# GStreamer/gst-plugins-rs

Measured on AMD Instinct MI355X. Metric: 4K RGBA frames/sec through hsvfilter+colorlut at 1 GPU; % HBM roofline, higher is better.
Workload: dtype u8

## Files before the change

gst-plugins-rs_amd/csrc/colorlut_kernels.hip:

```cpp
#include "internal.hpp"
#include "hsv_device.hpp"
#include "exact_math.hpp"

#include <cmath>
#include <cstring>
#include <map>
#include <memory>
#include <mutex>
#include <vector>

namespace mi355 {

struct LutK {
  float scale[3];
  float offset[3];
  int size;
};


__device__ __forceinline__ uint32_t floor_idx(float x, uint32_t max_idx) {
  const float f = floorf(x);
  uint32_t i = (f > 0.0f) ? ((f >= 4294967040.0f) ? 0xffffffffu : (uint32_t)f) : 0u;
  return i < max_idx ? i : max_idx;
}
// ... 825 lines not shown
  __shared__ uint32_t s_strip[4][512];
  s_spread[threadIdx.x] = spread3(threadIdx.x);
  __syncthreads();
  auto index = [&](uint32_t p) -> uint32_t { return s_spread[p & 0xffu] | (s_spread[(p >> 8) & 0xffu] << 1) | (s_spread[(p >> 16) & 0xffu] << 2); };
  const unsigned wave = threadIdx.x >> 6, lane = threadIdx.x & 63;
  uint32_t *x = s_strip[wave];
  const unsigned frame = blockIdx.x / tiles_per_frame, t = blockIdx.x - frame * tiles_per_frame;
  const u32x4_t *s4 = (const u32x4_t *)srcs.p[frame];
  u32x4_t *d4 = (u32x4_t *)dsts.p[frame];
  auto wave_sync = [] {
    __builtin_amdgcn_fence(__ATOMIC_ACQ_REL, "wavefront");
    __builtin_amdgcn_wave_barrier();
  };
  constexpr unsigned RPL = 64 / TW4;
  const unsigned sub = lane / TW4, g = lane % TW4;
  const unsigned tx = t % n_cols, ty = t / n_cols;
  const unsigned col = tx * TW4 + g;
  const unsigned r0 = ty * (8 * RPL) + wave * (2 * RPL) + sub, r1 = r0 + RPL;
  const bool ok0 = col < w4 && r0 < rows, ok1 = col < w4 && r1 < rows;
  const size_t i0 = (size_t)r0 * w4 + col, i1 = (size_t)r1 * w4 + col;
  u32x4_t p = {0, 0, 0, 0}, q = {0, 0, 0, 0};
  if (ok0) p = __builtin_nontemporal_load(s4 + i0);
  if (ok1) q = __builtin_nontemporal_load(s4 + i1);
  *(u32x4_t *)(x + lane * 4) = p;
  *(u32x4_t *)(x + 256 + lane * 4) = q;
  wave_sync();
  uint32_t px[8], o[8];
#pragma unroll
  for (int j = 0; j < 8; j++) px[j] = x[j * 64 + lane];
#pragma unroll
  for (int j = 0; j < 8; j++) o[j] = table[index(px[j])];
#pragma unroll
  for (int j = 0; j < 8; j++) x[j * 64 + lane] = (o[j] & 0x00ffffffu) | (px[j] & 0xff000000u);
  wave_sync();
  const u32x4_t r0v = *(u32x4_t *)(x + lane * 4), r1v = *(u32x4_t *)(x + 256 + lane * 4);
  if (ok0) __builtin_nontemporal_store(r0v, d4 + i0);
  if (ok1) __builtin_nontemporal_store(r1v, d4 + i1);
}

void shared_table_release(mi355_ctx *ctx, std::shared_ptr<void> *ref);
void lut_release(mi355_ctx *ctx) {
  for (int i = 0; i < 2; i++) {
    shared_table_release(ctx, &ctx->lut.table_ref[i]);
    if (ctx->lut.pick[i].ev0) (void)hipEventDestroy(ctx->lut.pick[i].ev0);
    if (ctx->lut.pick[i].ev1) (void)hipEventDestroy(ctx->lut.pick[i].ev1);
  }
// ... 713 lines not shown
  MultiFramePtrs s{}, d{};
  for (int f = 0; f < n_frames; f++) {
    if (!srcs[f] || !dsts[f] || (uintptr_t)srcs[f] % 16 != 0 || (uintptr_t)dsts[f] % 16 != 0) return MI355_ERR_UNSUPPORTED;
    s.p[f] = srcs[f];
    d.p[f] = dsts[f];
  }
  const unsigned w4 = (unsigned)width / 4;
  if (from_hbm && ctx->lut_variant == 0 && window_multi_applicable(ctx, w4, (size_t)height, n_frames)) {
    ctx->lut.last_kernel = "colorlut_window_kernel";
    return launch_window_table_multi(ctx, stream, table, srcs, dsts, n_frames, w4, (size_t)height);
  }
  ctx->lut.last_kernel = "colorlut_table_tiled_multi_kernel";
  const unsigned pad64 = (w4 + 63) / 64 * 64 - w4, pad32 = (w4 + 31) / 32 * 32 - w4;
  const unsigned tw4 = pad64 <= pad32 ? 64 : 32;
  const unsigned n_cols = (w4 + tw4 - 1) / tw4, rpb = 8 * (64 / tw4);
  const size_t tiles_per_frame = (size_t)n_cols * (((size_t)height + rpb - 1) / rpb);
  const size_t grid = tiles_per_frame * (size_t)n_frames;
  if (grid >= (1u << 31)) return MI355_ERR_UNSUPPORTED;
  if (tw4 == 64) hipLaunchKernelGGL((colorlut_table_tiled_multi_kernel<64>), dim3((unsigned)grid), dim3(256), 0, stream, s, d, w4, (unsigned)height, n_cols, (unsigned)tiles_per_frame, table);
  else hipLaunchKernelGGL((colorlut_table_tiled_multi_kernel<32>), dim3((unsigned)grid), dim3(256), 0, stream, s, d, w4, (unsigned)height, n_cols, (unsigned)tiles_per_frame, table);
  return check_hip(ctx, hipGetLastError(), "colorlut multi-frame table kernel launch");
}

void hsv_table_release(mi355_ctx *ctx) {
  HsvTable &T = ctx->hsv_table;
  shared_table_release(ctx, &T.table_ref);
  if (T.pick.ev0) (void)hipEventDestroy(T.pick.ev0);
  if (T.pick.ev1) (void)hipEventDestroy(T.pick.ev1);
  T = HsvTable{};
}

static int hsv_table_ensure(mi355_ctx *ctx, const PixFmt &fmt, const mi355_hsv_settings &hs) {
  HsvTable &T = ctx->hsv_table;
  if (T.valid && T.bgr == fmt.bgr && same_hs(T.hs, hs)) return MI355_OK;
  T.valid = false;
  T.d_table = nullptr;
  std::string key("H");
  key.push_back((char)('0' + fmt.bgr));
  key.append((const char *)&hs, sizeof(hs));
  int rc = shared_table_acquire(ctx, key, &T.table_ref, &T.d_table, [&](uint32_t *tab) {
    hipLaunchKernelGGL(table_domain_kernel, dim3(kTableEntries / 256), dim3(256), 0, ctx->stream, tab, 1);
    return launch_hsvfilter_compute(ctx, (uint8_t *)tab, 1, 0, 4096, 4096, 4096 * 4, fmt, hs);
  });
  if (rc) { T.table_ref.reset(); T.d_table = nullptr; return rc; }
  T.valid = true;
  T.bgr = fmt.bgr;
// ... 67 lines not shown
```

gst-plugins-rs_amd/csrc/group.hip:

```cpp
#include "internal.hpp"

#include <chrono>
#include <condition_variable>
#include <algorithm>
#include <cstring>
#include <deque>
#include <mutex>
#include <unordered_map>
#include <vector>

using namespace mi355;

namespace {

struct Desc {
  mi355_ctx *ctx;
  uint8_t *src, *dst;
  int width, height, stride, format;
  mi355_hsv_settings hs;
  const uint32_t *table;
  std::shared_ptr<void> table_ref;
  bool batchable;
  bool fused;
  uint64_t ticket;
// ... 715 lines not shown
    for (Set &s : sets) {
      (void)hipEventDestroy(s.done);
      kind.blocks.give(&s.data.block);
    }
    sets.clear();
    for (Item &d : pending)
      if (d.ready) (void)hipEventDestroy(d.ready);
    pending.clear();
    kind.destroy();
  }
};

}

struct mi355_group : GroupCore {
  int max_batch = 8;
  hipStream_t stream = nullptr;
  std::vector<Desc> pending;
  std::deque<Batch> batches;
  std::unordered_map<uint64_t, uint64_t> where;
  std::unordered_map<uint64_t, int> failed;
  uint64_t next_seq = 1;
  uint64_t n_frames = 0, n_batched_launch_pairs = 0, n_single = 0;
  std::vector<std::shared_ptr<void>> dead_refs;
  SetQueue<CmpKind> cmp;
  SetQueue<CdKind> cd;
  SetQueue<HdKind> hd;
  SetQueue<YdKind> yd;
  SetQueue<HnKind> hn;
  SetQueue<HfKind> hf;
};

namespace {

struct Locked {
  std::vector<std::shared_ptr<void>> reap;
  mi355_group *g;
  std::unique_lock<std::mutex> lk;
  explicit Locked(mi355_group *g_) : g(g_), lk(g_->mu) {}
  ~Locked() {
    if (!lk.owns_lock()) lk.lock();
    reap.swap(g->dead_refs);
    lk.unlock();
  }
};

void retire_front(mi355_group *g) {
  Batch &b = g->batches.front();
  for (uint64_t t : b.tickets) g->where.erase(t);
  g->events.push_back(b.done);
  if (b.table_ref) g->dead_refs.push_back(std::move(b.table_ref));
  g->batches.pop_front();
}

void retire_done(mi355_group *g) {
  while (!g->batches.empty() && g->batches.front().waiters == 0) {
    if (hipEventQuery(g->batches.front().done) != hipSuccess) { (void)hipGetLastError(); break; }
    retire_front(g);
  }
}

bool same_class(const Desc &a, const Desc &b) {
  return a.batchable && b.batchable && a.fused == b.fused && a.width == b.width && a.height == b.height && a.stride == b.stride && a.format == b.format && a.table == b.table &&
         std::memcmp(&a.hs, &b.hs, sizeof(a.hs)) == 0 && a.ctx->force_generic == b.ctx->force_generic;
}

int flush_locked(mi355_group *g, uint64_t until = 0) {
  bool reached = false;
  while (!g->pending.empty() && !reached) {
    std::vector<Desc> take, keep;
    std::vector<mi355_ctx *> blocked;
    const Desc first = g->pending.front();
    for (const Desc &d : g->pending) {
      bool stream_blocked = false;
      for (mi355_ctx *c : blocked) stream_blocked |= c == d.ctx;
      const bool fits = take.empty() || (!stream_blocked && (int)take.size() < g->max_batch && same_class(first, d));
      if (fits) take.push_back(d);
      else keep.push_back(d);
      if (!stream_blocked) blocked.push_back(d.ctx);
    }
    g->pending.swap(keep);
    PixFmt fmt;
    (void)pixfmt_of(first.format, &fmt);
    hipEvent_t done = take_event(g);
    if (!done) return fail(g, MI355_ERR_HIP, "hipEventCreate");
    int rc = MI355_OK;
    if (first.batchable) {
      uint8_t *srcs[kMultiFrames], *dsts[kMultiFrames];
      for (size_t i = 0; i < take.size(); i++) {
        srcs[i] = take[i].src;
        dsts[i] = take[i].dst;
        if (take[i].ready && hipStreamWaitEvent(g->stream, take[i].ready, 0) != hipSuccess) rc = MI355_ERR_HIP;
      }
      if (!rc && !first.fused) rc = launch_hsvfilter_multi(first.ctx, g->stream, srcs, (int)take.size(), first.width, first.height, fmt, first.hs);
      if (!rc) rc = launch_colorlut_multi(first.ctx, g->stream, first.table, srcs, dsts, (int)take.size(), first.width, first.height, first.fused);
      if (!rc && hipEventRecord(done, g->stream) != hipSuccess) rc = MI355_ERR_HIP;
      g->n_batched_launch_pairs++;
    } else {
      const Desc &d = take[0];
      const size_t pitch = (size_t)d.stride * (size_t)d.height;
      if (!g->batches.empty() && hipStreamWaitEvent(d.ctx->stream, g->batches.back().done, 0) != hipSuccess) rc = MI355_ERR_HIP;
      if (!rc && d.fused) rc = launch_hsv_colorlut(d.ctx, d.src, pitch, d.stride, d.dst, pitch, d.stride, 1, d.width, d.height, d.hs);
      if (!rc && !d.fused) rc = launch_hsvfilter(d.ctx, d.src, 1, pitch, d.width, d.height, d.stride, fmt, d.hs);
      if (!rc && !d.fused) rc = launch_colorlut(d.ctx, d.src, pitch, d.stride, d.dst, pitch, d.stride, 1, d.width, d.height, d.format);
      if (!rc && hipEventRecord(done, d.ctx->stream) != hipSuccess) rc = MI355_ERR_HIP;
      if (!rc && hipStreamWaitEvent(g->stream, done, 0) != hipSuccess) rc = MI355_ERR_HIP;
      if (rc && rc != MI355_ERR_HIP) g->last_error = d.ctx->last_error;
      g->n_single++;
    }
    for (const Desc &d : take)
      if (d.ready) g->events.push_back(d.ready);
    if (rc) {
      (void)hipGetLastError();
      g->events.push_back(done);
      if (g->failed.size() > 65536) g->failed.clear();
      for (const Desc &d : take) g->failed[d.ticket] = rc;
      if (g->last_error.empty()) g->last_error = "group launch failed";
      return rc;
// ... 572 lines not shown
  }
  return mi355_group_flush(g);
}

int mi355_group_submit_round_fused(mi355_group *g, mi355_ctx *const *ctxs, int n_streams, uint8_t *const *d_src, uint8_t *const *d_dst, int width,
                                   int height, int stride, int format, const mi355_hsv_settings *settings) {
  if (!g || !ctxs || !d_src || !d_dst || n_streams < 0) return MI355_ERR_INVALID_ARG;
  for (int i = 0; i < n_streams; i++) {
    int rc = mi355_group_submit_fused(g, ctxs[i], d_src[i], d_dst[i], width, height, stride, format, settings, nullptr);
    if (rc) return rc;
  }
  return mi355_group_flush(g);
}

int mi355_group_stats(mi355_group *g, uint64_t stats[3]) {
  if (!g || !stats) return MI355_ERR_INVALID_ARG;
  std::lock_guard<std::mutex> lk(g->mu);
  stats[0] = g->n_frames;
  stats[1] = g->n_batched_launch_pairs;
  stats[2] = g->n_single;
  return MI355_OK;
}

}

namespace {
std::mutex g_pg_mu;
struct ProcessGroup { int device; mi355_group *g; int refs; };
std::vector<ProcessGroup> g_pg;
}

extern "C" {

mi355_group *mi355_group_shared(int device, int *status) {
  std::lock_guard<std::mutex> lk(g_pg_mu);
  for (ProcessGroup &p : g_pg)
    if (p.device == device) { p.refs++; if (status) *status = MI355_OK; return p.g; }
  mi355_group *g = mi355_group_create(device, 0, status);
  if (g) g_pg.push_back(ProcessGroup{device, g, 1});
  return g;
}

void mi355_group_release(mi355_group *g) {
  if (!g) return;
  bool last = false;
  {
// ... 13 lines not shown
```

gst-plugins-rs_amd/csrc/hsv_device.hpp:

```cpp
#pragma once
#include "internal.hpp"
#include "exact_math.hpp"

namespace mi355 {

struct HsvK {
  float hue_shift, sat_mul, sat_off, val_mul, val_off;
};


template <bool FAST>
__device__ __forceinline__ void hsv_from_rgb(float r8, float g8, float b8, float &hue, float &sat,
                                             float &val) {
  if constexpr (FAST) {
    const float r = div255_u8(r8), g = div255_u8(g8), b = div255_u8(b8);
    const float value = fmaxf(fmaxf(r, g), b);
    const float minv = fminf(fminf(r, g), b);
    const float chroma = value - minv;
    const bool is_r = (r == value);
    const bool is_g = (g == value);
    const float na = is_r ? g : (is_g ? b : r);
    const float nb = is_r ? b : (is_g ? r : g);
    const float add = is_r ? 0.0f : (is_g ? 2.0f : 4.0f);
    const float q = div_rcp_refine(na - nb, fmaxf(chroma, 1e-30f));
// ... 289 lines not shown
    r = (r >= 360.0f) ? r - 360.0f : r;
    return __builtin_copysignf(r, t);
  }
  return fmodf(t, 360.0f);
}
template <int RPOS, int GPOS, int BPOS, int NPOS>
__device__ __forceinline__ void hsvfilter_px2_generic(uint32_t &p0, uint32_t &p1, const HsvK &k, const HsvLds *lds) {
  f2 h2, sat, value;
  hsv_from_rgb_pair_fast<RPOS, GPOS, BPOS, 1>(p0, p1, h2, sat, value, lds);
  uint32_t *px[2] = {&p0, &p1};
#pragma unroll
  for (int j = 0; j < 2; j++) {
    float h = hsv_fmod360_any((j ? h2.y : h2.x) + k.hue_shift);
    if (h < 0.0f) h += 360.0f;
    const float s = fminf(fmaxf(k.sat_mul * (j ? sat.y : sat.x) + k.sat_off, 0.0f), 1.0f);
    const float v = fminf(fmaxf(k.val_mul * (j ? value.y : value.x) + k.val_off, 0.0f), 1.0f);
    uint32_t r, g, b;
    hsv_to_rgb_generic(h, s, v, r, g, b);
    const uint32_t keep = *px[j] & (0xffu << (8 * NPOS));
    *px[j] = keep | (r << (8 * RPOS)) | (g << (8 * GPOS)) | (b << (8 * BPOS));
  }
}

inline int hsv_variant_for(const mi355_hsv_settings &s, bool force_generic, bool allow_wide = false) {
  const float a = fabsf(s.hue_shift);
  const bool narrow = (s.hue_shift == 0.0f) || (a >= 1e-30f && a <= 360.0f);
  const bool wide = allow_wide && a > 360.0f && a <= 4194304.0f;
  if (!(narrow || wide) || force_generic) return -1;
  const bool sv_ident = s.saturation_mul == 1.0f && s.saturation_off == 0.0f && s.value_mul == 1.0f && s.value_off == 0.0f;
  if (wide) return 8 | (s.hue_shift < 0.0f ? 1 : 0) | (sv_ident ? 4 : 0);
  const int shift = s.hue_shift == 0.0f ? HSV_SHIFT_ZERO : (s.hue_shift > 0.0f ? HSV_SHIFT_POS : HSV_SHIFT_NEG);
  return shift | (sv_ident ? 4 : 0);
}

}
```

gst-plugins-rs_amd/csrc/hsv_kernels.hip:

```cpp
#include "internal.hpp"
#include "exact_math.hpp"
#include "hsv_device.hpp"

namespace mi355 {


template <int VARIANT, int RPOS, int GPOS, int BPOS, int NPOS>
__device__ __forceinline__ void hsvfilter_quad(uint32_t &a, uint32_t &b, uint32_t &c, uint32_t &d, const HsvK &k, const HsvLds *lds) {
  if constexpr (VARIANT >= 0) {
    hsvfilter_px2_lds<RPOS, GPOS, BPOS, NPOS, hsv_shift_of(VARIANT), hsv_sv_ident_of(VARIANT)>(a, b, k, lds);
    hsvfilter_px2_lds<RPOS, GPOS, BPOS, NPOS, hsv_shift_of(VARIANT), hsv_sv_ident_of(VARIANT)>(c, d, k, lds);
  } else {
    hsvfilter_px2_generic<RPOS, GPOS, BPOS, NPOS>(a, b, k, lds);
    hsvfilter_px2_generic<RPOS, GPOS, BPOS, NPOS>(c, d, k, lds);
  }
}

template <int VARIANT, int FIRST, bool BGR>
__global__ __launch_bounds__(256) void hsvfilter_flat_kernel(uint4 *__restrict__ data, size_t n_vec,
                                                             HsvK k, int nt) {
  constexpr int RPOS = FIRST + (BGR ? 2 : 0), GPOS = FIRST + 1, BPOS = FIRST + (BGR ? 0 : 2);
  constexpr int NPOS = FIRST == 0 ? 3 : 0;
  __shared__ HsvLds lds;
  hsv_lds_fill<RPOS, GPOS, BPOS, NPOS>(&lds);
  __syncthreads();
  const size_t stride = (size_t)gridDim.x * blockDim.x;
  if (nt) {
    typedef uint32_t u32x4_t __attribute__((ext_vector_type(4)));
    u32x4_t *d4 = (u32x4_t *)data;
    for (size_t i = (size_t)blockIdx.x * blockDim.x + threadIdx.x; i < n_vec; i += stride) {
      const u32x4_t v = __builtin_nontemporal_load(d4 + i);
      uint4 p = {v.x, v.y, v.z, v.w};
      hsvfilter_quad<VARIANT, RPOS, GPOS, BPOS, NPOS>(p.x, p.y, p.z, p.w, k, &lds);
      const u32x4_t o = {p.x, p.y, p.z, p.w};
      __builtin_nontemporal_store(o, d4 + i);
    }
    return;
  }
  for (size_t i = (size_t)blockIdx.x * blockDim.x + threadIdx.x; i < n_vec; i += stride) {
// ... 161 lines not shown
    const size_t f = i / per_frame;
    const size_t r = i - f * per_frame;
    const size_t row = r / (size_t)width;
    const size_t col = r - row * (size_t)width;
    uint8_t *px = data + f * frame_pitch + row * (size_t)stride + col * (size_t)pixel_stride + first;
    const uint32_t c0 = px[0], c1 = px[1], c2 = px[2];
    const uint32_t p = bgr ? (c2 | (c1 << 8) | (c0 << 16)) : (c0 | (c1 << 8) | (c2 << 16));
    const uint32_t o = hsvfilter_px<FAST, 0, 1, 2, 3>(p, k, sel_tab);
    const uint8_t orr = (uint8_t)(o & 0xff), og = (uint8_t)((o >> 8) & 0xff), ob = (uint8_t)((o >> 16) & 0xff);
    px[0] = bgr ? ob : orr;
    px[1] = og;
    px[2] = bgr ? orr : ob;
  }
}

static int grid_for(mi355_ctx *ctx, size_t work_items, int block, int blocks_per_cu) {
  size_t blocks = (work_items + (size_t)block - 1) / (size_t)block;
  size_t cap = (size_t)ctx->n_cu * (size_t)blocks_per_cu;
  if (blocks > cap) blocks = cap;
  if (blocks < 1) blocks = 1;
  return (int)blocks;
}


template <class F>
static void with_variant(int variant, F &&f) {
  switch (variant) {
    case -1: f(std::integral_constant<int, -1>{}); break;
    case 0: f(std::integral_constant<int, 0>{}); break;
    case 1: f(std::integral_constant<int, 1>{}); break;
    case 2: f(std::integral_constant<int, 2>{}); break;
    case 4: f(std::integral_constant<int, 4>{}); break;
    case 5: f(std::integral_constant<int, 5>{}); break;
    case 6: f(std::integral_constant<int, 6>{}); break;
    case 8: f(std::integral_constant<int, 8>{}); break;
    case 9: f(std::integral_constant<int, 9>{}); break;
    case 12: f(std::integral_constant<int, 12>{}); break;
    default: f(std::integral_constant<int, 13>{}); break;
  }
}

template <class F>
static void with_flag(bool on, F &&f) {
  if (on) f(std::true_type{});
  else f(std::false_type{});
}

template <class F>
static void with_byte_order(int first, int bgr, F &&f) {
  if (first == 0 && !bgr) f(std::integral_constant<int, 0>{}, std::false_type{});
  else if (first == 0 && bgr) f(std::integral_constant<int, 0>{}, std::true_type{});
  else if (first == 1 && !bgr) f(std::integral_constant<int, 1>{}, std::false_type{});
  else f(std::integral_constant<int, 1>{}, std::true_type{});
}

static void launch_flat(mi355_ctx *ctx, int variant, uint4 *d, size_t n_vec, const HsvK &k, int first, int bgr, int grid) {
  const int nt = ctx->hsv_nt;
  with_variant(variant, [&](auto V) { with_byte_order(first, bgr, [&](auto FIRST, auto BGR) {
    hipLaunchKernelGGL((hsvfilter_flat_kernel<V, FIRST, BGR>), dim3(grid), dim3(256), 0, ctx->stream, d, n_vec, k, nt);
  }); });
}

static void launch_strided(mi355_ctx *ctx, int variant, uint8_t *d, int n_frames, size_t frame_pitch, int width, int height, int stride, const HsvK &k,
// ... 658 lines not shown
```

gst-plugins-rs_amd/csrc/internal.hpp:

```cpp
#pragma once
#include <hip/hip_runtime.h>
#include <cstddef>
#include <cstdint>
#include <cstring>
#include <memory>
#include <string>
#include <vector>
#include "../../include/mi355fx.h"

#include "autopick.hpp"
#include "colorlut_brick.hpp"
#include "colorlut_window.hpp"

namespace mi355 {

struct AutoPick : AutoPolicy {
  hipEvent_t ev0 = nullptr, ev1 = nullptr;
};

constexpr unsigned kStableCalls = 8;
struct Settled {
  mi355_hsv_settings hs{};
  int bgr = 0;
  unsigned stable = 0;
// ... 146 lines not shown
      (void)hipGetLastError();
      p = nullptr;
      return e;
    }
    n = want;
    return hipSuccess;
  }
};
template <typename T> using DeviceBuf = GrowBuf<T, false>;
template <typename T> using PinnedBuf = GrowBuf<T, true>;

int launch_hsvfilter(mi355_ctx *ctx, uint8_t *d_data, int n_frames, size_t frame_pitch, int width,
                     int height, int stride, const PixFmt &fmt, const mi355_hsv_settings &s);
int launch_hsvfilter_compute(mi355_ctx *ctx, uint8_t *d_data, int n_frames, size_t frame_pitch, int width,
                     int height, int stride, const PixFmt &fmt, const mi355_hsv_settings &s);
void hsv_table_release(mi355_ctx *ctx);
bool hsvfilter_multi_applicable(const uint8_t *const *frames, int n_frames, int width, int height, int stride, const PixFmt &fmt);
int launch_hsvfilter_multi(mi355_ctx *ctx, hipStream_t stream, uint8_t *const *frames, int n_frames, int width, int height, const PixFmt &fmt,
                           const mi355_hsv_settings &s);
int colorlut_multi_table(mi355_ctx *ctx, const uint32_t **table_out);
int colorlut_multi_fused_table(mi355_ctx *ctx, const mi355_hsv_settings *hs, const uint32_t **table_out);
int launch_colorlut_multi(mi355_ctx *ctx, hipStream_t stream, const uint32_t *table, uint8_t *const *srcs, uint8_t *const *dsts, int n_frames, int width,
                          int height, bool from_hbm = false);
int launch_hsvdetect(mi355_ctx *ctx, const uint8_t *d_src, size_t src_pitch, int src_stride,
                     const PixFmt &sfmt, uint8_t *d_dst, size_t dst_pitch, int dst_stride,
                     int dst_alpha_first, int dst_bgr, int n_frames, int width, int height,
                     const mi355_hsvdetect_settings &s);
int launch_colorlut(mi355_ctx *ctx, const uint8_t *d_src, size_t src_pitch, int src_stride,
                    uint8_t *d_dst, size_t dst_pitch, int dst_stride, int n_frames, int width,
                    int height, int format);
int launch_hsv_colorlut(mi355_ctx *ctx, const uint8_t *d_src, size_t src_pitch, int src_stride,
                        uint8_t *d_dst, size_t dst_pitch, int dst_stride, int n_frames, int width,
                        int height, const mi355_hsv_settings &hs);
bool table_variant(int lut_variant);
int lut_upload(mi355_ctx *ctx, int is3d, size_t size, const float *table, const float scale[3],
               const float offset[3]);
void lut_release(mi355_ctx *ctx);
int echo_setup(mi355_ctx *ctx, int n_streams, size_t ring_len);
void echo_release(mi355_ctx *ctx);
int launch_echo_batch(mi355_ctx *ctx, void *d_data, size_t stream_stride, size_t n, int is_f64, const size_t *delay, const double *intensity,
                      const double *feedback);
int launch_echo(mi355_ctx *ctx, void *d_data, size_t n, int is_f64, size_t delay, double intensity,
                double feedback);
int ebur128_setup(mi355_ctx *ctx, unsigned channels, unsigned rate, unsigned mode, const int *channel_class);
int ebur128_setup_batch(mi355_ctx *ctx, unsigned n_streams, unsigned channels, unsigned rate, unsigned mode, const int *channel_class);
int ebur128_add_frames_batch(mi355_ctx *ctx, const void *data, size_t frames, int fmt, int device_data);
// ... 246 lines not shown
```

gst-plugins-rs_amd/mi355fx/__init__.py:

```python
import ctypes as C
import os

import numpy as np

_HERE = os.path.dirname(os.path.abspath(__file__))
PKG_ROOT = os.path.dirname(_HERE)
LIB_PATH = os.environ.get("MI355FX_LIB") or os.path.join(PKG_ROOT, "libmi355fx.so")
HEADER_PATH = os.path.join(os.path.dirname(PKG_ROOT), "include", "mi355fx.h")

FMT = {"RGBx": 0, "xRGB": 1, "BGRx": 2, "xBGR": 3, "RGBA": 4, "ARGB": 5, "BGRA": 6, "ABGR": 7,
       "RGB": 8, "BGR": 9, "RGBA64_LE": 10, "RGBA64_BE": 11}
FMT_LAYOUT = {"RGBx": (4, 0, 0), "RGBA": (4, 0, 0), "RGB": (3, 0, 0), "xRGB": (4, 1, 0), "ARGB": (4, 1, 0),
              "BGRx": (4, 0, 1), "BGRA": (4, 0, 1), "BGR": (3, 0, 1), "xBGR": (4, 1, 1), "ABGR": (4, 1, 1)}

OK, ERR_INVALID_ARG, ERR_NO_DEVICE, ERR_HIP, ERR_NOT_CONFIGURED, ERR_OOM, ERR_UNSUPPORTED, ERR_TIMEOUT = 0, -1, -2, -3, -4, -5, -6, -7
FLAG_FORCE_GENERIC = 1
FLAG_HSV_BLOCKS_PER_CU = 2
FLAG_FUSED_VARIANT = 3
FLAG_LUT_VARIANT = 4
FLAG_LUT_STAGGER = 5
FLAG_HSV_TABLE = 6
FLAG_BRICK_TILES_PER_RUN = 7
FLAG_BRICK_SETS = 8
FLAG_BRICK_PRIO = 9
# ... 281 lines not shown
        "mi355_pipe_wait": (i, [vp, C.c_uint64]),
        "mi355_pipe_wait_all": (i, [vp]),
        "mi355_videocompare_hash_frame": (i, [vp, u8p, i, i, i, i, i, C.POINTER(C.c_uint64)]),
        "mi355_videocompare_hash_frames_device": (i, [vp, u8p, sz, i, i, i, i, i, i, C.POINTER(C.c_uint64)]),
        "mi355_videocompare_distance": (C.c_double, [i, C.c_uint64, C.c_uint64]),
        "mi355_dssim_create_image": (i, [vp, u8p, i, i, i, i, C.POINTER(vp)]),
        "mi355_dssim_create_image_device": (i, [vp, u8p, i, i, i, i, C.POINTER(vp)]),
        "mi355_dssim_free_image": (None, [vp, vp]),
        "mi355_dssim_compare": (i, [vp, vp, vp, C.POINTER(C.c_double)]),
        "mi355_dssim_compare_frames": (i, [vp, vp, C.POINTER(vp), i, i, i, i, i, C.POINTER(C.c_double)]),
        "mi355_dssim_compare_frames_device": (i, [vp, vp, C.POINTER(vp), i, i, i, i, i, C.POINTER(C.c_double)]),
        "mi355_issue_streams_round": (i, [C.POINTER(vp), i, C.POINTER(vp), C.POINTER(vp), i, i, i, i, C.POINTER(HsvSettings)]),
        "mi355_group_create": (vp, [i, i, C.POINTER(C.c_int)]),
        "mi355_group_destroy": (None, [vp]),
        "mi355_group_last_error": (C.c_char_p, [vp]),
        "mi355_group_submit_chain": (i, [vp, vp, u8p, u8p, i, i, i, i, C.POINTER(HsvSettings), C.POINTER(C.c_uint64)]),
        "mi355_group_submit_fused": (i, [vp, vp, u8p, u8p, i, i, i, i, C.POINTER(HsvSettings), C.POINTER(C.c_uint64)]),
        "mi355_group_flush": (i, [vp]),
        "mi355_pipe_set_group": (i, [vp, vp]),
        "mi355_group_wait": (i, [vp, C.c_uint64]),
        "mi355_group_order_after": (i, [vp, vp, C.c_uint64]),
        "mi355_group_wait_all": (i, [vp]),
        "mi355_group_stats": (i, [vp, C.POINTER(C.c_uint64)]),
        "mi355_group_set_rendezvous": (i, [vp, i, C.c_uint]),
        "mi355_group_set_compare_lanes": (i, [vp, i]),
        "mi355_group_submit_compare": (i, [vp, vp, u8p, u8p, i, i, i, i, i, C.POINTER(C.c_uint64)]),
        "mi355_group_wait_compare": (i, [vp, C.c_uint64, C.POINTER(C.c_double), C.POINTER(C.c_uint64)]),
        "mi355_group_compare_stats": (i, [vp, C.POINTER(C.c_uint64)]),
        "mi355_group_set_colordetect_rendezvous": (i, [vp, i, C.c_uint]),
        "mi355_group_submit_colordetect": (i, [vp, vp, vp, sz, i, i, i, C.POINTER(C.c_uint64)]),
        "mi355_group_wait_colordetect": (i, [vp, C.c_uint64, u8p, C.POINTER(C.c_int)]),
        "mi355_group_colordetect_stats": (i, [vp, C.POINTER(C.c_uint64)]),
        "mi355_selftest_colordetect_plan": (i, [i, i, C.POINTER(C.c_uint64), C.POINTER(C.c_uint32), C.POINTER(C.c_uint32), C.POINTER(C.c_uint64),
                                                C.POINTER(C.c_uint32)]),
        "mi355_group_set_hsvdetect_rendezvous": (i, [vp, i, C.c_uint]),
        "mi355_group_submit_hsvdetect": (i, [vp, vp, u8p, i, i, u8p, i, i, i, i, C.POINTER(HsvDetectSettings), C.POINTER(C.c_uint64)]),
        "mi355_group_wait_hsvdetect": (i, [vp, C.c_uint64]),
        "mi355_group_hsvdetect_stats": (i, [vp, C.POINTER(C.c_uint64)]),
        "mi355_selftest_hsvdetect_plan": (i, [i, i, C.c_uint, i, C.POINTER(C.c_uint64), C.POINTER(C.c_uint32), C.POINTER(C.c_uint32),
                                              C.POINTER(C.c_uint32)]),
        "mi355_group_set_hsvfilter_rendezvous": (i, [vp, i, C.c_uint]),
        "mi355_group_submit_hsvfilter": (i, [vp, vp, u8p, i, i, i, i, C.POINTER(HsvSettings), C.POINTER(C.c_uint64)]),
        "mi355_group_wait_hsvfilter": (i, [vp, C.c_uint64]),
        "mi355_group_hsvfilter_stats": (i, [vp, C.POINTER(C.c_uint64)]),
        "mi355_selftest_hsvfilter_set_plan": (i, [i, C.POINTER(HsvFilterPlanFrame), i, C.POINTER(HsvFilterPlanOut), C.POINTER(C.c_int)]),
        "mi355_agroup_create_echo": (vp, [i, i, sz, C.POINTER(C.c_int)]),
# ... 266 lines not shown
            n = len(contexts)
            arr = self._rounds[key] = ((C.c_void_p * n)(*[c.h for c in contexts]), (C.c_void_p * n)(*src_ptrs), (C.c_void_p * n)(*dst_ptrs))
        hs = HsvSettings(*[float(v) for v in settings])
        fn = self.L.mi355_group_submit_round_fused if fused else self.L.mi355_group_submit_round
        self._ck(fn(self.h, arr[0], len(contexts), arr[1], arr[2], width, height, stride, FMT[fmt], C.byref(hs)))

    def flush(self):
        self._ck(self.L.mi355_group_flush(self.h))

    def wait(self, ticket):
        self._ck(self.L.mi355_group_wait(self.h, ticket))

    def order_after(self, ctx, ticket):
        self._ck(self.L.mi355_group_order_after(self.h, ctx.h, ticket))

    def wait_all(self):
        self._ck(self.L.mi355_group_wait_all(self.h))

    def stats(self):
        c = (C.c_uint64 * 3)()
        self._ck(self.L.mi355_group_stats(self.h, c))
        return int(c[0]), int(c[1]), int(c[2])

    def set_rendezvous(self, expected_streams, linger_us):
        self._ck(self.L.mi355_group_set_rendezvous(self.h, expected_streams, linger_us))

    def set_compare_lanes(self, lanes):
        self._ck(self.L.mi355_group_set_compare_lanes(self.h, lanes))

    def submit_compare(self, ctx, d_ref, d_frame, stride, width, height, fmt="RGBA", algo=5):
        t = C.c_uint64(0)
        self._ck(self.L.mi355_group_submit_compare(self.h, ctx.h, d_ref, d_frame, stride, width, height, FMT[fmt], algo, C.byref(t)))
        return t.value

    def wait_compare(self, ticket):
        d = C.c_double(0.0)
        h = (C.c_uint64 * 2)()
        self._ck(self.L.mi355_group_wait_compare(self.h, ticket, C.byref(d), h))
        return d.value, int(h[0]), int(h[1])

    def compare_stats(self):
        c = (C.c_uint64 * 3)()
        self._ck(self.L.mi355_group_compare_stats(self.h, c))
        return int(c[0]), int(c[1]), int(c[2])

    def set_colordetect_rendezvous(self, expected_streams, linger_us):
# ... 1399 lines not shown
```

include/mi355fx.h:

```cpp
#ifndef MI355FX_H
#define MI355FX_H

#include <stddef.h>
#include <stdint.h>

#ifdef __cplusplus
extern "C" {
#endif

#define MI355FX_ABI_VERSION 1

typedef enum mi355_status {
  MI355_OK = 0,
  MI355_ERR_INVALID_ARG = -1,
  MI355_ERR_NO_DEVICE = -2,
  MI355_ERR_HIP = -3,
  MI355_ERR_NOT_CONFIGURED = -4,
  MI355_ERR_OUT_OF_MEMORY = -5,
  MI355_ERR_UNSUPPORTED = -6,
  MI355_ERR_TIMEOUT = -7
} mi355_status;

typedef enum mi355_video_format {
  MI355_FMT_RGBX = 0,
// ... 92 lines not shown
                            int *kind_out, int *measured_out);
int mi355_colorlut_frame(mi355_ctx *ctx, const uint8_t *src, int src_stride, uint8_t *dst,
                         int dst_stride, int width, int height, int format);
int mi355_colorlut_frames_device(mi355_ctx *ctx, const uint8_t *d_src, size_t src_pitch,
                                 int src_stride, uint8_t *d_dst, size_t dst_pitch, int dst_stride,
                                 int n_frames, int width, int height, int format);

int mi355_issue_streams_round(mi355_ctx *const *ctxs, int n_streams, uint8_t *const *d_src, uint8_t *const *d_dst,
                              int width, int height, int stride, int format, const mi355_hsv_settings *settings);

typedef struct mi355_group mi355_group;
mi355_group *mi355_group_create(int device, int max_batch, int *status);
void mi355_group_destroy(mi355_group *group);
const char *mi355_group_last_error(mi355_group *group);
int mi355_group_submit_chain(mi355_group *group, mi355_ctx *ctx, uint8_t *d_src, uint8_t *d_dst, int width, int height,
                             int stride, int format, const mi355_hsv_settings *settings, uint64_t *ticket);
int mi355_group_submit_fused(mi355_group *group, mi355_ctx *ctx, uint8_t *d_src, uint8_t *d_dst, int width, int height,
                             int stride, int format, const mi355_hsv_settings *settings, uint64_t *ticket);
int mi355_group_flush(mi355_group *group);
int mi355_group_order_after(mi355_group *group, mi355_ctx *ctx, uint64_t ticket);
int mi355_group_wait(mi355_group *group, uint64_t ticket);
int mi355_group_wait_all(mi355_group *group);
int mi355_group_stats(mi355_group *group, uint64_t stats[3]);
int mi355_group_submit_round(mi355_group *group, mi355_ctx *const *ctxs, int n_streams, uint8_t *const *d_src,
                             uint8_t *const *d_dst, int width, int height, int stride, int format,
                             const mi355_hsv_settings *settings);
int mi355_group_submit_round_fused(mi355_group *group, mi355_ctx *const *ctxs, int n_streams, uint8_t *const *d_src,
                                   uint8_t *const *d_dst, int width, int height, int stride, int format,
                                   const mi355_hsv_settings *settings);

int mi355_group_set_rendezvous(mi355_group *group, int expected_streams, unsigned linger_us);
int mi355_group_set_compare_lanes(mi355_group *group, int lanes);
int mi355_group_submit_compare(mi355_group *group, mi355_ctx *ctx, const uint8_t *d_ref, const uint8_t *d_frame, int stride, int width, int height,
                               int format, int algo, uint64_t *ticket);
int mi355_group_wait_compare(mi355_group *group, uint64_t ticket, double *distance, uint64_t hashes[2]);
int mi355_group_compare_stats(mi355_group *group, uint64_t stats[3]);

#define MI355_COLORDETECT_SET_MAX 32
int mi355_group_set_colordetect_rendezvous(mi355_group *group, int expected_streams, unsigned linger_us);
int mi355_group_submit_colordetect(mi355_group *group, mi355_ctx *ctx, const uint8_t *d_data, size_t data_len, int format, int quality,
                                   int max_colors, uint64_t *ticket);
int mi355_group_wait_colordetect(mi355_group *group, uint64_t ticket, uint8_t palette_rgb[255 * 3], int *n_colors);
int mi355_group_colordetect_stats(mi355_group *group, uint64_t stats[4]);
int mi355_selftest_colordetect_plan(int n_cu, int n_jobs, const uint64_t *n_samples, uint32_t *first_block, uint32_t *blocks,
                                    uint64_t *samples_per_block, uint32_t *total_blocks);

// ... 493 lines not shown
```

Measured before the change: 44320.

## Fuse hsvfilter and colorlut into one multi-frame chain kernel

Adds a kernel that applies the HSV filter and then the colour LUT to each tile inside a single launch. Previously the HSV pass wrote frames to HBM and the LUT pass read them back. The fused kernel still writes the HSV result back to the source buffer, which preserves the old in-place side effect. So it saves one full-frame read and one launch, and adds LDS table setup per block. It is used only when source and destination buffers do not overlap, and otherwise falls back to the two-launch path.

```diff
diff --git a/gst-plugins-rs_amd/csrc/colorlut_kernels.hip b/gst-plugins-rs_amd/csrc/colorlut_kernels.hip
--- a/gst-plugins-rs_amd/csrc/colorlut_kernels.hip
+++ b/gst-plugins-rs_amd/csrc/colorlut_kernels.hip
@@ -871,6 +871,60 @@
   u32x4_t p = {0, 0, 0, 0}, q = {0, 0, 0, 0};
   if (ok0) p = __builtin_nontemporal_load(s4 + i0);
   if (ok1) q = __builtin_nontemporal_load(s4 + i1);
+  *(u32x4_t *)(x + lane * 4) = p;
+  *(u32x4_t *)(x + 256 + lane * 4) = q;
+  wave_sync();
+  uint32_t px[8], o[8];
+#pragma unroll
+  for (int j = 0; j < 8; j++) px[j] = x[j * 64 + lane];
+#pragma unroll
+  for (int j = 0; j < 8; j++) o[j] = table[index(px[j])];
+#pragma unroll
+  for (int j = 0; j < 8; j++) x[j * 64 + lane] = (o[j] & 0x00ffffffu) | (px[j] & 0xff000000u);
+  wave_sync();
+  const u32x4_t r0v = *(u32x4_t *)(x + lane * 4), r1v = *(u32x4_t *)(x + 256 + lane * 4);
+  if (ok0) __builtin_nontemporal_store(r0v, d4 + i0);
+  if (ok1) __builtin_nontemporal_store(r1v, d4 + i1);
+}
+
+template <int VARIANT, int TW4>
+__global__ __launch_bounds__(256) void hsv_colorlut_chain_multi_kernel(MultiFramePtrs srcs, MultiFramePtrs dsts, unsigned w4, unsigned rows, unsigned n_cols,
+                                                                       unsigned tiles_per_frame, const uint32_t *__restrict__ table, HsvK k) {
+  __shared__ uint32_t s_spread[256];
+  __shared__ uint32_t s_strip[4][512];
+  __shared__ u32x4_t s_hsv[256];
+  static_assert(sizeof(s_hsv) == sizeof(HsvLdsImage), "one load per thread");
+  const unsigned wave = threadIdx.x >> 6, lane = threadIdx.x & 63;
+  uint32_t *x = s_strip[wave];
+  const unsigned frame = blockIdx.x / tiles_per_frame, t = blockIdx.x - frame * tiles_per_frame;
+  u32x4_t *s4 = (u32x4_t *)srcs.p[frame];
+  u32x4_t *d4 = (u32x4_t *)dsts.p[frame];
+  constexpr unsigned RPL = 64 / TW4;
+  const unsigned sub = lane / TW4, g = lane % TW4;
+  const unsigned tx = t % n_cols, ty = t / n_cols;
+  const unsigned col = tx * TW4 + g;
+  const unsigned r0 = ty * (8 * RPL) + wave * (2 * RPL) + sub, r1 = r0 + RPL;
+  const bool ok0 = col < w4 && r0 < rows, ok1 = col < w4 && r1 < rows;
+  const size_t i0 = (size_t)r0 * w4 + col, i1 = (size_t)r1 * w4 + col;
+  u32x4_t p = {0, 0, 0, 0}, q = {0, 0, 0, 0};
+  if (ok0) p = __builtin_nontemporal_load(s4 + i0);
+  if (ok1) q = __builtin_nontemporal_load(s4 + i1);
+  s_hsv[threadIdx.x] = ((const u32x4_t *)g_hsv_lds_image_rgba.words)[threadIdx.x];
+  s_spread[threadIdx.x] = spread3(threadIdx.x);
+  __syncthreads();
+  auto index = [&](uint32_t c) -> uint32_t { return s_spread[c & 0xffu] | (s_spread[(c >> 8) & 0xffu] << 1) | (s_spread[(c >> 16) & 0xffu] << 2); };
+  auto wave_sync = [] {
+    __builtin_amdgcn_fence(__ATOMIC_ACQ_REL, "wavefront");
+    __builtin_amdgcn_wave_barrier();
+  };
+  const HsvLds *lds = (const HsvLds *)s_hsv;
+  uint32_t f[8] = {p.x, p.y, p.z, p.w, q.x, q.y, q.z, q.w};
+  hsvfilter_quad<VARIANT, 0, 1, 2, 3>(f[0], f[1], f[2], f[3], k, lds);
+  hsvfilter_quad<VARIANT, 0, 1, 2, 3>(f[4], f[5], f[6], f[7], k, lds);
+  p = u32x4_t{f[0], f[1], f[2], f[3]};
+  q = u32x4_t{f[4], f[5], f[6], f[7]};
+  if (ok0) s4[i0] = p;
+  if (ok1) s4[i1] = q;
   *(u32x4_t *)(x + lane * 4) = p;
   *(u32x4_t *)(x + 256 + lane * 4) = q;
   wave_sync();
@@ -1630,6 +1684,33 @@
   return check_hip(ctx, hipGetLastError(), "colorlut multi-frame table kernel launch");
 }
 
+int launch_chain_multi(mi355_ctx *ctx, hipStream_t stream, const uint32_t *table, uint8_t *const *srcs, uint8_t *const *dsts, int n_frames, int width,
+                       int height, const PixFmt &fmt, const mi355_hsv_settings &hs) {
+  if (n_frames < 1 || n_frames > kMultiFrames || width % 4 != 0 || width < 128 || height <= 0) return MI355_ERR_UNSUPPORTED;
+  if (fmt.pixel_stride != 4 || fmt.first != 0 || fmt.bgr || !table) return MI355_ERR_UNSUPPORTED;
+  MultiFramePtrs s{}, d{};
+  for (int f = 0; f < n_frames; f++) {
+    if (!srcs[f] || !dsts[f] || (uintptr_t)srcs[f] % 16 != 0 || (uintptr_t)dsts[f] % 16 != 0) return MI355_ERR_UNSUPPORTED;
+    s.p[f] = srcs[f];
+    d.p[f] = dsts[f];
+  }
+  const HsvK k{hs.hue_shift, hs.saturation_mul, hs.saturation_off, hs.value_mul, hs.value_off};
+  const int variant = hsv_variant_for(hs, ctx->force_generic, true);
+  const unsigned w4 = (unsigned)width / 4;
+  const unsigned pad64 = (w4 + 63) / 64 * 64 - w4, pad32 = (w4 + 31) / 32 * 32 - w4;
+  const unsigned tw4 = pad64 <= pad32 ? 64 : 32;
+  const unsigned n_cols = (w4 + tw4 - 1) / tw4, rpb = 8 * (64 / tw4);
+  const size_t tiles_per_frame = (size_t)n_cols * (((size_t)height + rpb - 1) / rpb);
+  const size_t grid = tiles_per_frame * (size_t)n_frames;
+  if (grid >= (1u << 31)) return MI355_ERR_UNSUPPORTED;
+  ctx->lut.last_kernel = "colorlut_table_tiled_multi_kernel";
+  with_variant(variant, [&](auto V) {
+    if (tw4 == 64) hipLaunchKernelGGL((hsv_colorlut_chain_multi_kernel<V, 64>), dim3((unsigned)grid), dim3(256), 0, stream, s, d, w4, (unsigned)height, n_cols, (unsigned)tiles_per_frame, table, k);
+    else hipLaunchKernelGGL((hsv_colorlut_chain_multi_kernel<V, 32>), dim3((unsigned)grid), dim3(256), 0, stream, s, d, w4, (unsigned)height, n_cols, (unsigned)tiles_per_frame, table, k);
+  });
+  return check_hip(ctx, hipGetLastError(), "hsvfilter ! colorlut chain kernel launch");
+}
+
 void hsv_table_release(mi355_ctx *ctx) {
   HsvTable &T = ctx->hsv_table;
   shared_table_release(ctx, &T.table_ref);
diff --git a/gst-plugins-rs_amd/csrc/group.hip b/gst-plugins-rs_amd/csrc/group.hip
--- a/gst-plugins-rs_amd/csrc/group.hip
+++ b/gst-plugins-rs_amd/csrc/group.hip
@@ -761,6 +761,8 @@
   std::unordered_map<uint64_t, int> failed;
   uint64_t next_seq = 1;
   uint64_t n_frames = 0, n_batched_launch_pairs = 0, n_single = 0;
+  bool chain_one_launch = true;
+  uint64_t n_chain_one_launches = 0;
   std::vector<std::shared_ptr<void>> dead_refs;
   SetQueue<CmpKind> cmp;
   SetQueue<CdKind> cd;
@@ -802,6 +804,16 @@
 bool same_class(const Desc &a, const Desc &b) {
   return a.batchable && b.batchable && a.fused == b.fused && a.width == b.width && a.height == b.height && a.stride == b.stride && a.format == b.format && a.table == b.table &&
          std::memcmp(&a.hs, &b.hs, sizeof(a.hs)) == 0 && a.ctx->force_generic == b.ctx->force_generic;
+}
+
+bool chain_buffers_disjoint(const std::vector<Desc> &take) {
+  const uintptr_t bytes = (uintptr_t)take[0].stride * (uintptr_t)take[0].height;
+  for (const Desc &a : take)
+    for (const Desc &b : take) {
+      const uintptr_t d = (uintptr_t)a.dst, s = (uintptr_t)b.src;
+      if (d < s + bytes && s < d + bytes) return false;
+    }
+  return true;
 }
 
 int flush_locked(mi355_group *g, uint64_t until = 0) {
@@ -831,8 +843,15 @@
         dsts[i] = take[i].dst;
         if (take[i].ready && hipStreamWaitEvent(g->stream, take[i].ready, 0) != hipSuccess) rc = MI355_ERR_HIP;
       }
-      if (!rc && !first.fused) rc = launch_hsvfilter_multi(first.ctx, g->stream, srcs, (int)take.size(), first.width, first.height, fmt, first.hs);
-      if (!rc) rc = launch_colorlut_multi(first.ctx, g->stream, first.table, srcs, dsts, (int)take.size(), first.width, first.height, first.fused);
+      bool one_launch = false;
+      if (!rc && !first.fused && g->chain_one_launch && chain_buffers_disjoint(take)) {
+        const int r = launch_chain_multi(first.ctx, g->stream, first.table, srcs, dsts, (int)take.size(), first.width, first.height, fmt, first.hs);
+        one_launch = r == MI355_OK;
+        if (r != MI355_OK && r != MI355_ERR_UNSUPPORTED) rc = r;
+      }
+      if (!rc && !first.fused && !one_launch) rc = launch_hsvfilter_multi(first.ctx, g->stream, srcs, (int)take.size(), first.width, first.height, fmt, first.hs);
+      if (!rc && !one_launch) rc = launch_colorlut_multi(first.ctx, g->stream, first.table, srcs, dsts, (int)take.size(), first.width, first.height, first.fused);
+      if (one_launch) g->n_chain_one_launches++;
       if (!rc && hipEventRecord(done, g->stream) != hipSuccess) rc = MI355_ERR_HIP;
       g->n_batched_launch_pairs++;
     } else {
@@ -1451,6 +1470,19 @@
   return MI355_OK;
 }
 
+int mi355_group_set_chain_one_launch(mi355_group *g, int on) {
+  if (!g || (on != 0 && on != 1)) return MI355_ERR_INVALID_ARG;
+  std::lock_guard<std::mutex> lk(g->mu);
+  g->chain_one_launch = on != 0;
+  return MI355_OK;
+}
+
+uint64_t mi355_group_chain_one_launches(mi355_group *g) {
+  if (!g) return 0;
+  std::lock_guard<std::mutex> lk(g->mu);
+  return g->n_chain_one_launches;
+}
+
 }
 
 namespace {
diff --git a/gst-plugins-rs_amd/csrc/hsv_device.hpp b/gst-plugins-rs_amd/csrc/hsv_device.hpp
--- a/gst-plugins-rs_amd/csrc/hsv_device.hpp
+++ b/gst-plugins-rs_amd/csrc/hsv_device.hpp
@@ -335,6 +335,36 @@
   }
 }
 
+template <int VARIANT, int RPOS, int GPOS, int BPOS, int NPOS>
+__device__ __forceinline__ void hsvfilter_quad(uint32_t &a, uint32_t &b, uint32_t &c, uint32_t &d, const HsvK &k, const HsvLds *lds) {
+  if constexpr (VARIANT >= 0) {
+    hsvfilter_px2_lds<RPOS, GPOS, BPOS, NPOS, hsv_shift_of(VARIANT), hsv_sv_ident_of(VARIANT)>(a, b, k, lds);
+    hsvfilter_px2_lds<RPOS, GPOS, BPOS, NPOS, hsv_shift_of(VARIANT), hsv_sv_ident_of(VARIANT)>(c, d, k, lds);
+  } else {
+    hsvfilter_px2_generic<RPOS, GPOS, BPOS, NPOS>(a, b, k, lds);
+    hsvfilter_px2_generic<RPOS, GPOS, BPOS, NPOS>(c, d, k, lds);
+  }
+}
+
+struct alignas(16) HsvLdsImage { uint32_t words[1024]; };
+static_assert(sizeof(HsvLds) <= sizeof(HsvLdsImage), "one 16-byte load per thread of a 256-thread block covers HsvLds");
+static_assert(offsetof(HsvLds, value) == 0 && offsetof(HsvLds, rcpv) == 288 * 4 && offsetof(HsvLds, sext) == 576 * 4 && sizeof(uint2) == 8,
+              "the word offsets of hsv_make_lds_image_rgba");
+constexpr HsvLdsImage hsv_make_lds_image_rgba() {
+  HsvLdsImage im{};
+  const HsvValueTab t = hsv_make_value_tab();
+  for (int n = 0; n < 256; n++) {
+    im.words[n] = __builtin_bit_cast(uint32_t, t.value[n]);
+    im.words[288 + n] = __builtin_bit_cast(uint32_t, t.rcpv[n]);
+  }
+  for (int k = 0; k < 7; k++) {
+    im.words[576 + 64 * k] = hsv_sel_entry_floor(k, 0, 1, 2, 3);
+    im.words[576 + 64 * k + 1] = __builtin_bit_cast(uint32_t, (float)(2 * (k >> 1) + 1));
+  }
+  return im;
+}
+__device__ const HsvLdsImage g_hsv_lds_image_rgba = hsv_make_lds_image_rgba();
+
 inline int hsv_variant_for(const mi355_hsv_settings &s, bool force_generic, bool allow_wide = false) {
   const float a = fabsf(s.hue_shift);
   const bool narrow = (s.hue_shift == 0.0f) || (a >= 1e-30f && a <= 360.0f);
@@ -346,4 +376,21 @@
   return shift | (sv_ident ? 4 : 0);
 }
 
-}
+template <class F>
+static void with_variant(int variant, F &&f) {
+  switch (variant) {
+    case -1: f(std::integral_constant<int, -1>{}); break;
+    case 0: f(std::integral_constant<int, 0>{}); break;
+    case 1: f(std::integral_constant<int, 1>{}); break;
+    case 2: f(std::integral_constant<int, 2>{}); break;
+    case 4: f(std::integral_constant<int, 4>{}); break;
+    case 5: f(std::integral_constant<int, 5>{}); break;
+    case 6: f(std::integral_constant<int, 6>{}); break;
+    case 8: f(std::integral_constant<int, 8>{}); break;
+    case 9: f(std::integral_constant<int, 9>{}); break;
+    case 12: f(std::integral_constant<int, 12>{}); break;
+    default: f(std::integral_constant<int, 13>{}); break;
+  }
+}
+
+}
diff --git a/gst-plugins-rs_amd/csrc/hsv_kernels.hip b/gst-plugins-rs_amd/csrc/hsv_kernels.hip
--- a/gst-plugins-rs_amd/csrc/hsv_kernels.hip
+++ b/gst-plugins-rs_amd/csrc/hsv_kernels.hip
@@ -4,17 +4,6 @@
 
 namespace mi355 {
 
-
-template <int VARIANT, int RPOS, int GPOS, int BPOS, int NPOS>
-__device__ __forceinline__ void hsvfilter_quad(uint32_t &a, uint32_t &b, uint32_t &c, uint32_t &d, const HsvK &k, const HsvLds *lds) {
-  if constexpr (VARIANT >= 0) {
-    hsvfilter_px2_lds<RPOS, GPOS, BPOS, NPOS, hsv_shift_of(VARIANT), hsv_sv_ident_of(VARIANT)>(a, b, k, lds);
-    hsvfilter_px2_lds<RPOS, GPOS, BPOS, NPOS, hsv_shift_of(VARIANT), hsv_sv_ident_of(VARIANT)>(c, d, k, lds);
-  } else {
-    hsvfilter_px2_generic<RPOS, GPOS, BPOS, NPOS>(a, b, k, lds);
-    hsvfilter_px2_generic<RPOS, GPOS, BPOS, NPOS>(c, d, k, lds);
-  }
-}
 
 template <int VARIANT, int FIRST, bool BGR>
 __global__ __launch_bounds__(256) void hsvfilter_flat_kernel(uint4 *__restrict__ data, size_t n_vec,
@@ -222,23 +211,6 @@
   return (int)blocks;
 }
 
-
-template <class F>
-static void with_variant(int variant, F &&f) {
-  switch (variant) {
-    case -1: f(std::integral_constant<int, -1>{}); break;
-    case 0: f(std::integral_constant<int, 0>{}); break;
-    case 1: f(std::integral_constant<int, 1>{}); break;
-    case 2: f(std::integral_constant<int, 2>{}); break;
-    case 4: f(std::integral_constant<int, 4>{}); break;
-    case 5: f(std::integral_constant<int, 5>{}); break;
-    case 6: f(std::integral_constant<int, 6>{}); break;
-    case 8: f(std::integral_constant<int, 8>{}); break;
-    case 9: f(std::integral_constant<int, 9>{}); break;
-    case 12: f(std::integral_constant<int, 12>{}); break;
-    default: f(std::integral_constant<int, 13>{}); break;
-  }
-}
 
 template <class F>
 static void with_flag(bool on, F &&f) {
diff --git a/gst-plugins-rs_amd/csrc/internal.hpp b/gst-plugins-rs_amd/csrc/internal.hpp
--- a/gst-plugins-rs_amd/csrc/internal.hpp
+++ b/gst-plugins-rs_amd/csrc/internal.hpp
@@ -192,6 +192,8 @@
 int colorlut_multi_fused_table(mi355_ctx *ctx, const mi355_hsv_settings *hs, const uint32_t **table_out);
 int launch_colorlut_multi(mi355_ctx *ctx, hipStream_t stream, const uint32_t *table, uint8_t *const *srcs, uint8_t *const *dsts, int n_frames, int width,
                           int height, bool from_hbm = false);
+int launch_chain_multi(mi355_ctx *ctx, hipStream_t stream, const uint32_t *table, uint8_t *const *srcs, uint8_t *const *dsts, int n_frames, int width,
+                       int height, const PixFmt &fmt, const mi355_hsv_settings &hs);
 int launch_hsvdetect(mi355_ctx *ctx, const uint8_t *d_src, size_t src_pitch, int src_stride,
                      const PixFmt &sfmt, uint8_t *d_dst, size_t dst_pitch, int dst_stride,
                      int dst_alpha_first, int dst_bgr, int n_frames, int width, int height,
diff --git a/gst-plugins-rs_amd/mi355fx/__init__.py b/gst-plugins-rs_amd/mi355fx/__init__.py
--- a/gst-plugins-rs_amd/mi355fx/__init__.py
+++ b/gst-plugins-rs_amd/mi355fx/__init__.py
@@ -327,6 +327,8 @@
         "mi355_group_order_after": (i, [vp, vp, C.c_uint64]),
         "mi355_group_wait_all": (i, [vp]),
         "mi355_group_stats": (i, [vp, C.POINTER(C.c_uint64)]),
+        "mi355_group_set_chain_one_launch": (i, [vp, i]),
+        "mi355_group_chain_one_launches": (C.c_uint64, [vp]),
         "mi355_group_set_rendezvous": (i, [vp, i, C.c_uint]),
         "mi355_group_set_compare_lanes": (i, [vp, i]),
         "mi355_group_submit_compare": (i, [vp, vp, u8p, u8p, i, i, i, i, i, C.POINTER(C.c_uint64)]),
@@ -639,6 +641,12 @@
         self._ck(self.L.mi355_group_stats(self.h, c))
         return int(c[0]), int(c[1]), int(c[2])
 
+    def set_chain_one_launch(self, on):
+        self._ck(self.L.mi355_group_set_chain_one_launch(self.h, 1 if on else 0))
+
+    def chain_one_launches(self):
+        return int(self.L.mi355_group_chain_one_launches(self.h))
+
     def set_rendezvous(self, expected_streams, linger_us):
         self._ck(self.L.mi355_group_set_rendezvous(self.h, expected_streams, linger_us))
 
diff --git a/include/mi355fx.h b/include/mi355fx.h
--- a/include/mi355fx.h
+++ b/include/mi355fx.h
@@ -138,6 +138,8 @@
 int mi355_group_wait(mi355_group *group, uint64_t ticket);
 int mi355_group_wait_all(mi355_group *group);
 int mi355_group_stats(mi355_group *group, uint64_t stats[3]);
+int mi355_group_set_chain_one_launch(mi355_group *group, int on);
+uint64_t mi355_group_chain_one_launches(mi355_group *group);
 int mi355_group_submit_round(mi355_group *group, mi355_ctx *const *ctxs, int n_streams, uint8_t *const *d_src,
                              uint8_t *const *d_dst, int width, int height, int stride, int format,
                              const mi355_hsv_settings *settings);
```

After: 44330, median of 2. Within noise of the previous version (+0.0%).
